# vaenyr/stable-diffusion-on-device

Hardware: AMD Instinct MI355X
Metric: images/sec + per-UNet-step ms, SD v1.4 512x512 20-step PLMS, 1/2/4/8 MI355X (higher is better)
Workload: dtype f16; 1 GPU; SD v1.4 txt2img 512x512, 20-step PLMS (21 UNet evals, batch 2 = cond+uncond per image), CLIP encode + VAE decode + uint8, guidance 7.5; images_per_gpu=1, global_batch=1, parallelism=dp1 (image shards, 1 RCCL broadcast), hip_graph=True, trajectory_graph=True, decode_overlaps_next_sampling=False

## Files before the change

include/sdod_engine.h:

```cpp
#ifndef SDOD_ENGINE_H
#define SDOD_ENGINE_H

#include <stddef.h>
#include <stdint.h>

#ifndef SDOD_API
#define SDOD_API
#endif

#ifdef __cplusplus
extern "C" {
#endif

enum sdod_graph_kind { SDOD_GRAPH_UNET = 0, SDOD_GRAPH_VAE_DECODER = 1, SDOD_GRAPH_TEXT_ENCODER = 2, SDOD_GRAPH_TEMB = 3,
                       SDOD_GRAPH_VAE_ENCODER = 4, SDOD_GRAPH_VAE_ENCODER_MASKED = 5 };

typedef struct sdod_model_config {
    int latent_channels;
    int latent_h;
    int latent_w;
    int model_channels;
    int context_dim;
    int context_len;
    int num_heads;
// ... 8 lines not shown
    int concat_channels;
} sdod_model_config;

SDOD_API void sdod_model_config_sd14(sdod_model_config* cfg);
SDOD_API void sdod_model_config_sd21(sdod_model_config* cfg);

SDOD_API int sdod_graph_create(void** graph, int kind, const sdod_model_config* cfg, int batch);
SDOD_API int sdod_graph_destroy(void* graph);

SDOD_API int sdod_graph_num_params(void* graph);
SDOD_API int sdod_graph_param_info(void* graph, int index, const char** name, int* ndim, int64_t shape[4]);
SDOD_API int sdod_graph_set_param(void* graph, const char* name, const void* data, int dtype, const int64_t* shape, int ndim);
SDOD_API int sdod_graph_param_device(void* graph, const char* name, void** device_ptr, size_t* bytes);
SDOD_API int sdod_graph_load_file(void* graph, const char* path, const char* prefix);
SDOD_API int sdod_graph_finalize(void* graph);
SDOD_API int sdod_graph_io(void* graph, int is_output, int index, void** device_ptr, size_t* bytes);
enum sdod_exec_flags { SDOD_EXEC_HIP_GRAPH = 1, SDOD_EXEC_STATIC_UNCHANGED = 2 };
SDOD_API int sdod_graph_execute(void* graph, void* stream, int flags);
SDOD_API int sdod_graph_check(void* graph);
SDOD_API int sdod_graph_num_ops(void* graph);
SDOD_API int sdod_graph_op_info(void* graph, int index, const char** label, double* flops, double* bytes);
SDOD_API int sdod_graph_op_detail(void* graph, int index, const char** detail);
SDOD_API int sdod_graph_profile(void* graph, void* stream, int iters, float* ms_out, int n);
SDOD_API int sdod_graph_stats(void* graph, size_t* weight_bytes, size_t* arena_bytes, int* num_launches, double* flops);
SDOD_API int sdod_graph_tune_info(void* graph, int* from_table, int* tuned_in_process, char* table_path, int cap);

#ifdef __cplusplus
}
#endif
#endif
// ... 1 lines not shown
```

include/sdod_hip.h:

```cpp
#ifndef SDOD_HIP_H
#define SDOD_HIP_H

#include <stddef.h>
#include <stdint.h>

#ifndef SDOD_API
#define SDOD_API
#endif

#ifdef __cplusplus
extern "C" {
#endif

enum sdod_act { SDOD_ACT_NONE = 0, SDOD_ACT_SILU = 1, SDOD_ACT_GELU = 2, SDOD_ACT_QUICK_GELU = 3 };
enum sdod_dtype { SDOD_F16 = 0, SDOD_F32 = 1, SDOD_U8Q = 2, SDOD_BF16 = 3  };
enum sdod_a_mode { SDOD_A_ROWS = 0, SDOD_A_CONV3X3 = 1  };

typedef struct sdod_gemm_desc {
    const void* a;
    const void* a2;
    const void* w;
    const void* bias;
    const void* row_bias;
    const void* residual;
// ... 181 lines not shown
    uint64_t seed, image_index0;
    int n, c, hw, uncond_first, mode, v_pred, last, noise_level, stage_reps, temb_width, temb_reps;
    float guidance, vc0, vc1, sqrt_one_minus_at, sqrt_at, sqrt_a_prev, dir_coef, known_sa, known_s1a;
} sdod_ddim_inpaint_step_args;
SDOD_API int sdod_ddim_inpaint_step(const sdod_ddim_inpaint_step_args* a, void* stream);
SDOD_API int sdod_mask_to_latent_f32(const uint8_t* mask_u8, float* keep, int n, int h_lat, int w_lat, int factor, void* stream);
SDOD_API int sdod_image_composite_u8(const void* img, const uint8_t* init_u8, const uint8_t* mask_u8, uint8_t* out_u8, int n, size_t hw,
                                     float a, float b, int mode, void* stream);
SDOD_API int sdod_image_to_u8(const void* img, uint8_t* out, size_t count, float a, float b, int mode, void* stream);

SDOD_API const char* sdod_hip_last_error(void);
SDOD_API int sdod_hip_device_info(int* cu_count, size_t* hbm_bytes, char* arch, int arch_len);

SDOD_API int sdod_l2_prefetch(const void* ptr, size_t bytes, void* stream);

#ifdef __cplusplus
}
#endif
#endif
```

stable-diffusion-on-device_amd/csrc/elementwise.hip:

```cpp
#include "common.h"
#include <atomic>
#include "sdod_hip.h"
#include "host_util.h"

#pragma clang fp contract(off)

namespace {

SDOD_DEVICE float mul_rn(float a, float b) { return a * b; }
SDOD_DEVICE float add_rn(float a, float b) { return a + b; }
SDOD_DEVICE float sub_rn(float a, float b) { return a - b; }
SDOD_DEVICE float div_rn(float a, float b) { return a / b; }

inline int grid_for(size_t work, int block = 256) {
    size_t b = (work + block - 1) / block;
    if (b > 2048) b = 2048;
    if (b < 1) b = 1;
    return (int)b;
}

#define GRID_STRIDE(i, n) \
    for (size_t i = (size_t)blockIdx.x * blockDim.x + threadIdx.x; i < (n); i += (size_t)gridDim.x * blockDim.x)

__global__ void geglu_kernel(const f16* x, f16* y, int M, int C) {
// ... 933 lines not shown
    SDOD_REQUIRE(out && e0 && count > 0 && div != 0.0f, "bad argument");
    LAUNCH(lincomb4_kernel, count, stream, out, e0, e1, e2, e3, c0, c1, c2, c3, div, count);
    return 0;
    SDOD_CATCH
}

extern "C" int sdod_image_to_u8(const void* img, uint8_t* out, size_t count, float a, float b, int mode, void* stream) {
    SDOD_TRY
    SDOD_REQUIRE(img && out && count > 0 && (mode == 0 || mode == 1), "bad argument");
    LAUNCH(to_u8_kernel, count, stream, (const f16*)img, out, count, a, b, mode);
    return 0;
    SDOD_CATCH
}

namespace {
__global__ __launch_bounds__(256) void l2_prefetch_kernel(const unsigned* __restrict__ p, size_t lines, unsigned* sink) {
    unsigned acc = 0;
    const size_t stride = (size_t)gridDim.x * blockDim.x;
    for (size_t i = (size_t)blockIdx.x * blockDim.x + threadIdx.x; i < lines; i += stride) acc += p[i * 32];
    if (acc == 0x9e3779b9u) *sink = acc;
}
}

extern "C" int sdod_l2_prefetch(const void* ptr, size_t bytes, void* stream) {
    SDOD_TRY
    SDOD_REQUIRE(ptr != nullptr && ((uintptr_t)ptr & 3) == 0, "null / unaligned pointer");
    const size_t lines = bytes / 128;
    if (lines == 0) return 0;
    static std::atomic<unsigned*> sink[64];
    int dev = 0;
// ... 16 lines not shown
```

stable-diffusion-on-device_amd/csrc/engine.h:

```cpp
#pragma once
#include <hip/hip_runtime.h>

#include <cstdint>
#include <functional>
#include <map>
#include <string>
#include <unordered_map>
#include <vector>

#include "host_util.h"
#include "sdod_engine.h"
#include "sdod_hip.h"

namespace sdod {

typedef _Float16 f16;

enum ParamKind {
    PK_CONV3,
    PK_CONV3_SMALL,
    PK_CONV1,
    PK_LINEAR,
    PK_EMBED,
    PK_VEC,
// ... 30 lines not shown
    void* ptr = nullptr;
    size_t bytes = 0;
};

class Graph {
public:
    Graph(int kind, const sdod_model_config& cfg, int batch);
    ~Graph();
    Graph(const Graph&) = delete;

    int num_params() const { return (int)params_.size(); }
    const Param& param(int i) const { return params_.at(i); }
    void set_param(const std::string& name, const void* data, int dtype, const int64_t* shape, int ndim);
    void load_file(const std::string& path, const std::string& prefix);
    void finalize();
    void execute(hipStream_t st, bool use_hip_graph, bool skip_static = false);
    void check_health() const;
    IoSlot io(bool output, int index) const;
    void stats(size_t* wbytes, size_t* abytes, int* launches, double* flops) const;

private:
    enum Mode { DECLARE, DRY, REAL };
    int kind_;
    sdod_model_config cfg_;
    int batch_;
    Mode mode_ = DECLARE;
    bool finalized_ = false;

    std::vector<Param> params_;
    std::unordered_map<std::string, int> pindex_;
    std::vector<std::vector<int>> groups_;
    std::unordered_map<std::string, int> gindex_;
    char* weight_base_ = nullptr;
    size_t weight_bytes_ = 0;
    float* qscale_ = nullptr;
    float* qoff_ = nullptr;
    size_t qrows_ = 0;
    bool quant_mode() const { return cfg_.weight_quant != 0 && (kind_ == SDOD_GRAPH_UNET || kind_ == SDOD_GRAPH_TEMB); }
    static constexpr int kQuantAutoMaxRows = 128;
    bool quant_decl_ = false;
    void quant_rows(int rows) { quant_decl_ = quant_mode() && (cfg_.weight_quant == 1 || rows <= kQuantAutoMaxRows); }
    void quant_global() { quant_decl_ = quant_mode(); }
// ... 89 lines not shown
        f16* c; const f16* p; int ld, n_out, n_mid, k;
        const float *bias_w, *bias_p;
        float* bias_out;
    };
    std::vector<ComposeJob> compose_jobs_;
    std::vector<void*> derived_;
    void emit_gemm(sdod_gemm_desc d);
    void linear(const f16* x, int rows, int K, int w, int N, f16* out, const GemmOpt& o);
    void linear_raw(const f16* x, int rows, int K, const f16* w, int ldw, int N, f16* out, const GemmOpt& o);
    Act conv(const Act& x, const Act* x2, int w, int cout, int ksize, int stride, bool upsample, const GemmOpt& o);
    Act group_norm(const Act& x, const Act* x2, int gw, int gb, float eps, bool silu);
    Act layer_norm(const Act& x, int lw, int lb, float eps);
    void attention(const f16* q, const f16* k, const f16* v, f16* out, int B, int heads, int lq, int lk, int d, int ldq,
                   int ldk, int ldv, int ldo, bool causal);

    Act res_block(const std::string& pfx, const Act& x, const Act* x2, int cout, const f16* emb_all, int emb_ld, int& emb_off);
    std::vector<Op>& sink() { return to_static_ ? static_ops_ : ops_; }
    struct PendingReduce {
        bool active = false;
        sdod_gemm_desc d{};
        double bytes = 0;
        std::string detail;
    } pending_;
    void flush_pending();
    std::vector<const void*> parked_;
    void release_after_consumer(const Act& a) { parked_.push_back(a.p); }
    void drain_parked() {
        for (const void* p : parked_) release(p);
        parked_.clear();
    }
    void settle() {
        flush_pending();
        drain_parked();
    }
    Act spatial_transformer(const std::string& pfx, const Act& x, const Act& ctx);
    Act vae_res_block(const std::string& pfx, const Act& x, int cout);
    Act vae_attn_block(const std::string& pfx, const Act& x);
    int emb_total_ = 0;
    int kv_total_ = 0;
    f16* kv_all_ = nullptr;
    int kv_off_ = 0;
    std::vector<std::pair<std::string, int>> unet_res_blocks() const;
    const char* group_base(const std::string& group) const;
    int group_first(const std::string& group) const;
    void emit(std::function<void(hipStream_t)> fn, const char* label = "elementwise", double flops = 0, double bytes = 0) {
        settle();
        if (mode_ == REAL) sink().push_back(Op{std::move(fn), label, flops, bytes, ""});
    }

public:
// ... 9 lines not shown
```

stable-diffusion-on-device_amd/csrc/engine.hip:

```cpp
#include "engine.h"

#include <cstdio>

#include <dlfcn.h>
#include <fcntl.h>
#include <sys/mman.h>
#include <sys/stat.h>
#include <unistd.h>

#include <algorithm>
#include <cstdlib>
#include <cstring>
#include <map>
#include <mutex>
#include <thread>

namespace sdod {

static inline size_t align_up(size_t v, size_t a) { return (v + a - 1) / a * a; }

static void check_rc(int rc) {
    if (rc != 0) throw Error(rc, get_last_error());
}

// ... 869 lines not shown
}

void Graph::build() {
    quant_global();
    switch (kind_) {
    case SDOD_GRAPH_UNET: build_unet(); break;
    case SDOD_GRAPH_VAE_DECODER: build_vae(); break;
    case SDOD_GRAPH_TEXT_ENCODER: build_clip(); break;
    case SDOD_GRAPH_VAE_ENCODER: build_vae_encoder(false); break;
    case SDOD_GRAPH_VAE_ENCODER_MASKED: build_vae_encoder(true); break;
    default: build_temb(); break;
    }
    settle();
}

void Graph::finalize() {
    allocate_weights();
    SDOD_REQUIRE(!finalized_, "graph already finalized");
    std::string missing;
    int nmiss = 0;
    for (auto& p : params_)
        if (!p.set) {
            if (nmiss < 5) missing += (nmiss ? ", " : "") + p.name;
            ++nmiss;
        }
    SDOD_REQUIRE(nmiss == 0, std::to_string(nmiss) + " parameter(s) not set: " + missing + (nmiss > 5 ? ", ..." : ""));
    mode_ = DRY;
    arena_reset();
    ws_need_ = gn_ws_need_ = 0;
    build();
// ... 244 lines not shown
    SDOD_TRY
    SDOD_REQUIRE(graph && path, "null argument");
    static_cast<Graph*>(graph)->load_file(path, prefix ? prefix : "");
    return 0;
    SDOD_CATCH
}

extern "C" int sdod_graph_finalize(void* graph) {
    SDOD_TRY
    SDOD_REQUIRE(graph != nullptr, "null graph");
    static_cast<Graph*>(graph)->finalize();
    return 0;
    SDOD_CATCH
}

extern "C" int sdod_graph_io(void* graph, int is_output, int index, void** device_ptr, size_t* bytes) {
    SDOD_TRY
    SDOD_REQUIRE(graph != nullptr, "null graph");
    const sdod::IoSlot s = static_cast<Graph*>(graph)->io(is_output != 0, index);
    if (device_ptr) *device_ptr = s.ptr;
    if (bytes) *bytes = s.bytes;
    return 0;
    SDOD_CATCH
}

extern "C" int sdod_graph_param_device(void* graph, const char* name, void** device_ptr, size_t* bytes) {
    SDOD_TRY
    SDOD_REQUIRE(graph != nullptr && name != nullptr, "null argument");
    Graph* g = static_cast<Graph*>(graph);
    for (int i = 0; i < g->num_params(); ++i) {
// ... 84 lines not shown
```

stable-diffusion-on-device_amd/csrc/graphs.hip:

```cpp
#include "engine.h"

namespace sdod {

static void check_rc2(int rc) {
    if (rc != 0) throw Error(rc, get_last_error());
}

int Graph::group_first(const std::string& group) const {
    auto it = gindex_.find(group);
    if (it == gindex_.end()) throw Error(INTERNAL_ERROR, "unknown parameter group " + group);
    return groups_[it->second].front();
}

const char* Graph::group_base(const std::string& group) const {
    auto it = gindex_.find(group);
    if (it == gindex_.end()) throw Error(INTERNAL_ERROR, "unknown parameter group " + group);
    return params_[groups_[it->second].front()].dev;
}

Act Graph::res_block(const std::string& pfx, const Act& x, const Act* x2, int cout, const f16* emb_all, int emb_ld, int& emb_off) {
    const int cin = x.c + (x2 ? x2->c : 0);
    quant_rows(x.rows());
    const int n1w = P(pfx + ".in_layers.0.weight", {cin}, PK_VEC), n1b = P(pfx + ".in_layers.0.bias", {cin}, PK_VEC);
    const int c1w = P(pfx + ".in_layers.2.weight", {cout, cin, 3, 3}, PK_CONV3), c1b = P(pfx + ".in_layers.2.bias", {cout}, PK_VEC);
    const int n2w = P(pfx + ".out_layers.0.weight", {cout}, PK_VEC), n2b = P(pfx + ".out_layers.0.bias", {cout}, PK_VEC);
    int c2w, skw = -1, skb = -1;
    const bool fuse_skip = !quant_decl_;
    if (cin != cout && !fuse_skip) {
        c2w = P(pfx + ".out_layers.3.weight", {cout, cout, 3, 3}, PK_CONV3);
        skw = P(pfx + ".skip_connection.weight", {cout, cin, 1, 1}, PK_CONV1);
        skb = P(pfx + ".skip_connection.bias", {cout}, PK_VEC);
    } else if (cin != cout) {
        const int ld = 9 * cout + cin;
        c2w = Pc(pfx + ".out_layers.3.weight", {cout, cout, 3, 3}, PK_CONV3, ld, 0, -1);
        skw = Pc(pfx + ".skip_connection.weight", {cout, cin, 1, 1}, PK_CONV1, ld, 9 * cout, c2w);
        skb = P(pfx + ".skip_connection.bias", {cout}, PK_VEC);
    } else {
// ... 4 lines not shown
    const int my_off = emb_off;
    emb_off += cout;

    Act g1 = group_norm(x, x2, n1w, n1b, 1e-5f, true);
    GemmOpt o1;
    o1.bias = c1b;
    o1.row_bias = emb_all ? emb_all + my_off : nullptr;
    o1.ld_row_bias = emb_ld;
    o1.rows_per_img = x.h * x.w;
    Act h = conv(g1, nullptr, c1w, cout, 3, 1, false, o1);
    release(g1);
    Act g2 = group_norm(h, nullptr, n2w, n2b, 1e-5f, true);
    release(h);
    GemmOpt o2;
    o2.bias = c2b;
    Act sk;
    if (cin != cout && !fuse_skip) {
        GemmOpt os;
        os.bias = skb;
        sk = conv(x, x2, skw, cout, 1, 1, false, os);
        o2.residual = sk.p;
    } else if (cin != cout) {
        o2.tail0 = &x;
        o2.tail1 = x2;
        o2.bias2 = skb;
    } else {
        if (x2) throw Error(INTERNAL_ERROR, "identity skip with a concatenated input");
        o2.residual = x.p;
    }
    Act out = conv(g2, nullptr, c2w, cout, 3, 1, false, o2);
    release(g2);
    if (sk.p) release_after_consumer(sk);
    return out;
}

Act Graph::spatial_transformer(const std::string& pfx, const Act& x, const Act& ctx) {
    const int C = x.c, cd = ctx.c;
    const int heads = cfg_.num_heads > 0 ? cfg_.num_heads : C / cfg_.head_dim;
    const int d = C / heads;
    const int rows = x.rows(), L = x.h * x.w, B = x.n;
    const std::string tb = pfx + ".transformer_blocks.0";
    quant_rows(rows);
    const bool quant_block = quant_decl_;
    const int nw = P(pfx + ".norm.weight", {C}, PK_VEC), nb = P(pfx + ".norm.bias", {C}, PK_VEC);
    const bool lin = cfg_.linear_proj != 0;
    const int piw = lin ? P(pfx + ".proj_in.weight", {C, C}, PK_LINEAR) : P(pfx + ".proj_in.weight", {C, C, 1, 1}, PK_CONV1);
    const int pib = P(pfx + ".proj_in.bias", {C}, PK_VEC);
    const int l1w = P(tb + ".norm1.weight", {C}, PK_VEC), l1b = P(tb + ".norm1.bias", {C}, PK_VEC);
    const std::string gq = tb + ".attn1.qkv";
    P(tb + ".attn1.to_q.weight", {C, C}, PK_LINEAR, gq);
    P(tb + ".attn1.to_k.weight", {C, C}, PK_LINEAR, gq);
// ... 13 lines not shown
    static const bool compose_on = [] { const char* e = std::getenv("SDOD_COMPOSE"); return !(e && e[0] == '0'); }();
    const bool compose = compose_on && !quant_block;
    int f2w, pow_;
    if (compose) {
        f2w = Pc(tb + ".ff.net.2.weight", {C, 4 * C}, PK_LINEAR, 5 * C, 0, -1);
        pow_ = lin ? Pc(pfx + ".proj_out.weight", {C, C}, PK_LINEAR, 5 * C, 4 * C, f2w)
                   : Pc(pfx + ".proj_out.weight", {C, C, 1, 1}, PK_CONV1, 5 * C, 4 * C, f2w);
    } else {
        f2w = P(tb + ".ff.net.2.weight", {C, 4 * C}, PK_LINEAR);
        pow_ = lin ? P(pfx + ".proj_out.weight", {C, C}, PK_LINEAR) : P(pfx + ".proj_out.weight", {C, C, 1, 1}, PK_CONV1);
    }
    const int f2b = P(tb + ".ff.net.2.bias", {C}, PK_VEC);
    const int pob = P(pfx + ".proj_out.bias", {C}, PK_VEC);
    if (mode_ == DECLARE) return act(x.n, x.h, x.w, C);

    Act g = group_norm(x, nullptr, nw, nb, 1e-6f, false);
    Act t0 = act(B, 1, L, C);
    { GemmOpt o; o.bias = pib; linear(g.p, rows, C, piw, C, t0.p, o); }
    release(g);
    const bool fold = !quant_block;
    auto normed = [&](const Act& src, int lw, int lb) -> Act { return layer_norm(src, lw, lb, 1e-5f); };
    f16* qkv = alloc((size_t)rows * 3 * C);
    if (fold) {
        GemmOpt o; o.ln_w = l1w; o.ln_b = l1b;
        linear_raw(t0.p, rows, C, reinterpret_cast<const f16*>(group_base(gq)), C, 3 * C, qkv, o);
    } else {
        Act nrm = normed(t0, l1w, l1b);
        GemmOpt o; o.wq_scale = qscale_of(group_first(gq)); o.wq_off = qoff_of(group_first(gq));
        linear_raw(nrm.p, rows, C, reinterpret_cast<const f16*>(group_base(gq)), C, 3 * C, qkv, o);
        release(nrm);
    }
    f16* a1 = alloc((size_t)rows * C);
    attention(qkv, qkv + C, qkv + 2 * C, a1, B, heads, L, L, d, 3 * C, 3 * C, 3 * C, C, false);
    release(qkv);
    Act t1 = act(B, 1, L, C);
    { GemmOpt o; o.bias = o1b; o.residual = t0.p; linear(a1, rows, C, o1w, C, t1.p, o); }
    release(a1); release(t0);
    static const bool xfold_on = [] { const char* e = std::getenv("SDOD_XATTN_FOLD"); return !(e && e[0] == '0'); }();
    const int NK = heads * 80;
    const bool xfold = xfold_on && fold && ctx.w <= 80 && NK % 320 == 0 && L % 32 == 0 && d <= 160 && d % 4 == 0;
    if (xfold) {
        f16 *w1 = nullptr, *w2 = nullptr;
        float *s1 = nullptr, *t1v = nullptr;
        f16* wq = reinterpret_cast<f16*>(params_[q2w].dev);
        const f16* wo = reinterpret_cast<const f16*>(params_[o2w].dev);
        if (mode_ == REAL) {
            SDOD_HIP_CHECK(hipMalloc((void**)&w1, (size_t)B * NK * C * sizeof(f16)));
            SDOD_HIP_CHECK(hipMalloc((void**)&w2, (size_t)B * NK * C * sizeof(f16)));
            SDOD_HIP_CHECK(hipMalloc((void**)&s1, (size_t)B * NK * sizeof(float)));
            SDOD_HIP_CHECK(hipMalloc((void**)&t1v, (size_t)B * NK * sizeof(float)));
            derived_.push_back(w1); derived_.push_back(w2); derived_.push_back(s1); derived_.push_back(t1v);
            const LnVecs qv = ln_fold_vectors(wq, C, C, C, l2w, l2b, nullptr);
// ... 161 lines not shown
                              "M" + std::to_string(B * H * Wd) + " N" + std::to_string(MC) + " K64"});
        }
    } else {
        f16* cols = alloc((size_t)B * H * Wd * 64);
        emit([=](hipStream_t st) { check_rc2(sdod_latent_im2col_f16(x_in, cols, B, H, Wd, LC, 64, 1.0f, st)); });
        { GemmOpt o; o.bias = cib; linear(cols, B * H * Wd, 64, ciw, MC, h.p, o); }
        release(cols);
    }

    std::vector<Act> hs;
    hs.push_back(h);
    int ch = MC, ds = 1, idx = 1;
    for (int level = 0; level < 4; ++level) {
        for (int i = 0; i < 2; ++i) {
            const std::string pfx = "input_blocks." + std::to_string(idx++);
            Act r = res_block(pfx + ".0", h, nullptr, mult[level] * MC, emb_all, emb_ld, emb_off);
            ch = mult[level] * MC;
            if (ds <= 4) {
                Act t = spatial_transformer(pfx + ".1", r, ctx);
                release(r);
                r = t;
            }
            h = r;
            hs.push_back(h);
        }
        if (level != 3) {
            const std::string pfx = "input_blocks." + std::to_string(idx++) + ".0.op";
            quant_rows(h.rows() / 4);
            const int w = P(pfx + ".weight", {ch, ch, 3, 3}, PK_CONV3), b = P(pfx + ".bias", {ch}, PK_VEC);
            GemmOpt o; o.bias = b;
            h = conv(h, nullptr, w, ch, 3, 2, false, o);
            hs.push_back(h);
            ds *= 2;
        }
// ... 356 lines not shown
```

stable-diffusion-on-device_amd/csrc/libsdod/context.cpp:

```cpp
#include "context.h"

#include <algorithm>
#include <cstdio>
#include <cstring>

#include "sdod_hip.h"

namespace sdod {

static void rc_check(int rc) {
    if (rc != 0) throw Error(rc, get_last_error());
}

void Logger::log(LogLevel l, const std::string& msg) const {
    if (l == LogLevel::NOTHING || (unsigned)l > (unsigned)level_) return;
    static const char* tag[] = {"", "E", "I", "D", "A"};
    std::FILE* sink = l == LogLevel::ERROR ? stderr : stdout;
    std::fprintf(sink, "[libsdod %s] %s\n", tag[(unsigned)l], msg.c_str());
    std::fflush(sink);
}

namespace {
struct Timer {
    std::chrono::steady_clock::time_point t0 = std::chrono::steady_clock::now();
// ... 30 lines not shown
    Timer t;
    tokenizer_.emplace(models_dir_ + "/ctokenizer.txt");
    logger_.info("Tokenizer created!");
    solver_.emplace(1000, 0.00085f, 0.0120f);
    logger_.info("ODE solver prepared!");
    SDOD_HIP_CHECK(hipSetDevice(device_));
    SDOD_HIP_CHECK(hipStreamCreateWithFlags(&stream_, hipStreamNonBlocking));

    struct Item { std::unique_ptr<Graph>* slot; int kind; int batch; const char* stem; };
    const Item items[] = {{&unet_, SDOD_GRAPH_UNET, 2, "unet"}, {&text_, SDOD_GRAPH_TEXT_ENCODER, 1, "text_encoder"},
                          {&vae_, SDOD_GRAPH_VAE_DECODER, 1, "vae_decoder"}};
    for (const Item& it : items) {
        logger_.info(std::string("Attempting to load a model: ") + it.stem + ".sdodw");
        it.slot->reset(new Graph(it.kind, cfg_, it.batch));
        (*it.slot)->load_file(weight_path(it.stem), "");
        (*it.slot)->finalize();
        logger_.info(std::string("Model ") + it.stem + " loaded");
    }
    logger_.info("All models loaded!");

    const size_t lat = (size_t)latent_channels_ * latent_spatial_ * latent_spatial_;
    SDOD_HIP_CHECK(hipMalloc((void**)&x_dev_, 2 * lat * sizeof(float)));
    SDOD_HIP_CHECK(hipMalloc((void**)&e_dev_, lat * sizeof(float)));
    SDOD_HIP_CHECK(hipMalloc((void**)&y_prev_, lat * sizeof(float)));
    SDOD_HIP_CHECK(hipMalloc((void**)&img_u8_, image_bytes()));
    SDOD_HIP_CHECK(hipMalloc((void**)&ctx_uncond_, (size_t)cfg_.context_len * cfg_.context_dim * sizeof(f16)));
    x_host_.resize(lat);

    encode_prompt("", ctx_uncond_);
    logger_.info("Input/output buffers created and prepared!");
// ... 129 lines not shown
```

stable-diffusion-on-device_amd/csrc/norms.hip:

```cpp
#include "common.h"
#include "sdod_hip.h"
#include "host_util.h"

#include <algorithm>
#include <cstdlib>

namespace {

struct GnMom {
    float n, mean, m2;
};
SDOD_DEVICE GnMom gn_merge(GnMom a, const GnMom& b) {
    if (b.n == 0.f) return a;
    if (a.n == 0.f) return b;
    const float n = a.n + b.n, d = b.mean - a.mean, f = b.n / n;
    a.mean += d * f;
    a.m2 += b.m2 + d * d * a.n * f;
    a.n = n;
    return a;
}

template <typename T>
struct Chunk8;
template <>
// ... 951 lines not shown
            if (pix < pix_end) {
                f16x8 o;
#pragma unroll
                for (int e = 0; e < 8; ++e) {
                    float f = (float)v[k][e] * s8[e] + t8[e];
                    if (p.silu) f = silu_f(f);
                    o[e] = (f16)f;
                }
                stg8(p.y + (row0 + pix) * p.C + c0, o);
            }
        }
    }
}

constexpr size_t GN_GRID_MIN_BYTES = (size_t)5 << 20;

static int gn_device_cus() {
    static std::atomic<int> cus[64];
    int dev = 0;
    if (hipGetDevice(&dev) != hipSuccess || dev < 0 || dev >= 64) return 0;
    int v = cus[dev].load(std::memory_order_relaxed);
    if (v == 0) {
        if (hipDeviceGetAttribute(&v, hipDeviceAttributeMultiprocessorCount, dev) != hipSuccess || v <= 0) v = -1;
        cus[dev].store(v, std::memory_order_relaxed);
    }
    return v > 0 ? v : 0;
}

static int gn_grid_plan(int n, int hw, int c0, int c1, int groups, GnGridP* out) {
    const int c = c0 + c1;
    if (groups > 32 || n <= 0 || !gn2_fits(c0, c1, groups) || c / 8 > 512) return 0;
    if ((size_t)n * hw * c * 2 < GN_GRID_MIN_BYTES) return 0;
    int cus = gn_device_cus();
    if (cus > 256) cus = 256;
    const int wpi = cus / n;
    if (wpi < 8 || wpi > GN_MAX_CHUNKS_GRID) return 0;
    const int cp = c / 8, rp = 512 / cp;
    const int ppw = (hw + wpi - 1) / wpi;
    const int k = (ppw + rp - 1) / rp;
    if (k > 16 * 8) return 0;
    if (out) {
        out->cp = cp; out->rp = rp; out->wpi = wpi; out->ppw = ppw; out->nwg = wpi * n;
        out->nloop = k <= 16 ? 1 : (k + 15) / 16;
    }
    return k <= 4 ? 4 : k <= 8 ? 8 : 16;
}

// ... 726 lines not shown
```

stable-diffusion-on-device_amd/sdod/amd/_lib.py:

```python
import ctypes
import os

_HERE = os.path.dirname(os.path.abspath(__file__))
LIB_DIR = os.path.normpath(os.path.join(_HERE, '..', '..', 'lib'))

_cache = {}


def load(name):
    if name in _cache:
        return _cache[name]
    path = os.path.join(LIB_DIR, os.environ.get('SDOD_LIBSDOD', name) if name == 'libsdod.so' else name)
    if not os.path.exists(path):
        raise ImportError(
            f'{path} not found: build the MI355X extension first '
            f'(python -c "import __graft_entry__ as g; g.build()" or make -C stable-diffusion-on-device_amd). '
            f'There is no CPU fallback for the HIP path.')
    lib = ctypes.CDLL(path, mode=ctypes.RTLD_GLOBAL)
    _cache[name] = lib
    return lib


class SdodError(RuntimeError):
    def __init__(self, code, msg):
# ... 105 lines not shown
        'sdod_ddim_inpaint_step': (c_int, [ctypes.POINTER(DdimInpaintStepArgs), P]),
        'sdod_mask_to_latent_f32': (c_int, [P, P, c_int, c_int, c_int, c_int, P]),
        'sdod_image_composite_u8': (c_int, [P, P, P, P, c_int, c_size_t, c_float, c_float, c_int, P]),
        'sdod_nchw_f32_to_nhwc_f16': (c_int, [P, P, c_int, c_int, c_int, c_float, P]),
        'sdod_nhwc_f16_to_nchw_f32': (c_int, [P, P, c_int, c_int, c_int, P]),
        'sdod_latent_prep_f16': (c_int, [P, P, P, P, c_int, c_int, c_int, c_float, P]),
        'sdod_embedding_f16': (c_int, [P, P, P, P, c_int, c_int, c_int, P]),
        'sdod_timestep_features_f16': (c_int, [P, P, c_int, c_int, P]),
        'sdod_stage_unet_inputs': (c_int, [P, P, c_size_t, c_int, P, P, c_size_t, c_int, P]),
        'sdod_randn_f32': (c_int, [P, P, c_size_t, ctypes.c_uint64, ctypes.c_uint64, P]),
        'sdod_cfg_combine': (c_int, [P, P, c_int, c_int, c_int, c_float, c_int, c_int, P]),
        'sdod_dpm_update': (c_int, [P, P, P, c_size_t, c_int, c_float, c_float, c_float, c_float, c_float, P]),
        'sdod_ddim_step_f32': (c_int, [P, P, c_size_t, c_float, c_float, c_float, c_float, P]),
        'sdod_lincomb4_f32': (c_int, [P, P, P, P, P, c_float, c_float, c_float, c_float, c_float, c_size_t, P]),
        'sdod_image_to_u8': (c_int, [P, P, c_size_t, c_float, c_float, c_int, P]),
        'sdod_hip_last_error': (c_char_p, []),
        'sdod_hip_device_info': (c_int, [ctypes.POINTER(c_int), ctypes.POINTER(c_size_t), c_char_p, c_int]),
    }
    for name, (res, args) in sig.items():
        fn = getattr(lib, name)
        fn.restype = res
        fn.argtypes = args


HIP_SYMBOLS = [
    'sdod_gemm_f16', 'sdod_gemm_fixup', 'sdod_gemm_fixup_counters', 'sdod_gemm_workspace_bytes', 'sdod_gemm_plan', 'sdod_gemm_halo_ok', 'sdod_gemm_panel_ok', 'sdod_gemm_xcd_panels', 'sdod_gemm_num_tiles', 'sdod_gemm_tile_shape', 'sdod_gemm_tile_info', 'sdod_gemm_time', 'sdod_gemm_time_cold', 'sdod_group_norm_workspace_bytes', 'sdod_group_norm_layout', 'sdod_group_norm_status', 'sdod_group_norm_clear_error', 'sdod_l2_prefetch', 'sdod_group_norm_launches', 'sdod_group_norm_path', 'sdod_group_norm_nhwc', 'sdod_group_norm_nchw', 'sdod_group_norm_nchw_workspace_bytes', 'sdod_gemm_reduce_info', 'sdod_group_norm_reduce_ok', 'sdod_group_norm_reduce_nhwc',
    'sdod_layer_norm_f16', 'sdod_ln_fold_f16', 'sdod_compose_linear_f16', 'sdod_attention_f16', 'sdod_xattn_fold_f16', 'sdod_softmax_rows_f16', 'sdod_geglu_f16', 'sdod_act_f16',
    'sdod_add_f16', 'sdod_concat_channels_f16', 'sdod_im2col3x3_small_f16', 'sdod_latent_im2col_f16', 'sdod_conv_in_f16', 'sdod_image_conv_in_f16', 'sdod_conv_in_cat_f16', 'sdod_masked_image_conv_in_f16', 'sdod_inpaint_cond_f32', 'sdod_encode_latent_f32', 'sdod_plms_update', 'sdod_dpm_step', 'sdod_ddim_inpaint_step', 'sdod_mask_to_latent_f32', 'sdod_image_composite_u8', 'sdod_nchw_f32_to_nhwc_f16',
    'sdod_nhwc_f16_to_nchw_f32', 'sdod_latent_prep_f16', 'sdod_embedding_f16', 'sdod_timestep_features_f16', 'sdod_cfg_combine', 'sdod_stage_unet_inputs', 'sdod_randn_f32',
    'sdod_dpm_update', 'sdod_ddim_step_f32', 'sdod_lincomb4_f32', 'sdod_image_to_u8', 'sdod_hip_last_error',
    'sdod_hip_device_info',
]


def check(code):
    if code != 0:
        msg = hip().sdod_hip_last_error()
        raise SdodError(code, msg.decode() if msg else 'unknown error')
```

stable-diffusion-on-device_amd/sdod/amd/engine.py:

```python
import contextlib
import ctypes

import numpy as np
import torch

from . import _lib
from ._lib import check

UNET, VAE_DECODER, TEXT_ENCODER, TEMB, VAE_ENCODER, VAE_ENCODER_MASKED = 0, 1, 2, 3, 4, 5


class ModelConfig(ctypes.Structure):
    _fields_ = [(n, ctypes.c_int) for n in (
        'latent_channels', 'latent_h', 'latent_w', 'model_channels', 'context_dim', 'context_len', 'num_heads',
        'head_dim', 'vocab_size', 'text_layers', 'text_heads', 'vae_channels', 'linear_proj', 'text_arch', 'weight_quant',
        'concat_channels')]


ENGINE_SYMBOLS = [
    'sdod_model_config_sd14', 'sdod_model_config_sd21', 'sdod_graph_create', 'sdod_graph_destroy', 'sdod_graph_num_params', 'sdod_graph_param_info',
    'sdod_graph_set_param', 'sdod_graph_param_device', 'sdod_graph_load_file', 'sdod_graph_finalize', 'sdod_graph_io', 'sdod_graph_execute', 'sdod_graph_check',
    'sdod_graph_stats', 'sdod_graph_tune_info', 'sdod_graph_num_ops', 'sdod_graph_op_info', 'sdod_graph_op_detail', 'sdod_graph_profile',
]


def _engine():
    lib = _lib.hip()
    if not getattr(lib, '_sdod_engine_typed', False):
        P, I = ctypes.c_void_p, ctypes.c_int
        lib.sdod_model_config_sd14.argtypes = [ctypes.POINTER(ModelConfig)]
        lib.sdod_model_config_sd14.restype = None
        lib.sdod_model_config_sd21.argtypes = [ctypes.POINTER(ModelConfig)]
        lib.sdod_model_config_sd21.restype = None
        lib.sdod_graph_create.argtypes = [ctypes.POINTER(P), I, ctypes.POINTER(ModelConfig), I]
        lib.sdod_graph_destroy.argtypes = [P]
        lib.sdod_graph_num_params.argtypes = [P]
        lib.sdod_graph_param_info.argtypes = [P, I, ctypes.POINTER(ctypes.c_char_p), ctypes.POINTER(I), ctypes.POINTER(ctypes.c_int64)]
        lib.sdod_graph_set_param.argtypes = [P, ctypes.c_char_p, P, I, ctypes.POINTER(ctypes.c_int64), I]
        lib.sdod_graph_load_file.argtypes = [P, ctypes.c_char_p, ctypes.c_char_p]
        lib.sdod_graph_param_device.argtypes = [P, ctypes.c_char_p, ctypes.POINTER(P), ctypes.POINTER(ctypes.c_size_t)]
        lib.sdod_graph_finalize.argtypes = [P]
        lib.sdod_graph_io.argtypes = [P, I, I, ctypes.POINTER(P), ctypes.POINTER(ctypes.c_size_t)]
        lib.sdod_graph_execute.argtypes = [P, P, I]
        lib.sdod_graph_check.argtypes = [P]
        lib.sdod_graph_stats.argtypes = [P, ctypes.POINTER(ctypes.c_size_t), ctypes.POINTER(ctypes.c_size_t), ctypes.POINTER(I),
                                         ctypes.POINTER(ctypes.c_double)]
        lib.sdod_graph_tune_info.argtypes = [P, ctypes.POINTER(I), ctypes.POINTER(I), ctypes.c_char_p, I]
        lib.sdod_graph_num_ops.argtypes = [P]
        lib.sdod_graph_op_info.argtypes = [P, I, ctypes.POINTER(ctypes.c_char_p), ctypes.POINTER(ctypes.c_double), ctypes.POINTER(ctypes.c_double)]
        lib.sdod_graph_profile.argtypes = [P, P, I, P, I]
        lib.sdod_graph_op_detail.argtypes = [P, I, ctypes.POINTER(ctypes.c_char_p)]
        lib._sdod_engine_typed = True
    return lib


def sd14_config(latent_h=64, latent_w=64, concat_channels=0):
# ... 69 lines not shown
        check(self._lib.sdod_graph_param_device(self._h, name.encode(), ctypes.byref(p), ctypes.byref(n)))
        return device_view(p.value, (n.value // torch.empty((), dtype=dtype).element_size(),), dtype, self.device)

    def load_state_dict(self, sd, prefix=''):
        with torch.cuda.device(self.device):
            for name, _ in self.param_table():
                key = prefix + name
                if key not in sd:
                    raise KeyError(f'missing parameter {key}')
                self.set_param(name, sd[key])

    def load_file(self, path, prefix=''):
        with self._on_device():
            check(self._lib.sdod_graph_load_file(self._h, path.encode(), prefix.encode()))

    def finalize(self):
        with torch.cuda.device(self.device):
            check(self._lib.sdod_graph_finalize(self._h))
        self.finalized = True
        return self

    def _io(self, is_out, idx):
        p = ctypes.c_void_p(); n = ctypes.c_size_t()
        check(self._lib.sdod_graph_io(self._h, 1 if is_out else 0, idx, ctypes.byref(p), ctypes.byref(n)))
        return p.value, n.value

    def io_tensor(self, is_out, idx, shape, dtype):
        ptr, nbytes = self._io(is_out, idx)
        numel = int(np.prod(shape))
        assert numel * torch.empty((), dtype=dtype).element_size() == nbytes, (shape, dtype, nbytes)
# ... 123 lines not shown
```

stable-diffusion-on-device_amd/sdod/amd/pipeline.py:

```python
import numpy as np
import torch

from . import engine as E
from . import ops
from .host import DpmSolver
from .samplers import PLMS_ORDERS, PlmsSchedule


class Txt2Img:
    inpaint_unet = False
    _cond_staged = False
    encoder = None
    masked_encoder = None
    _traj = None

    def __init__(self, state_dicts=None, models_dir=None, images_per_gpu=1, latent_hw=64, device='cuda:0', use_hip_graph=True,
                 tokenizer=None, with_text_encoder=True, model='sd14', with_vae=True, cfg_split=False, weight_quant=None,
                 with_vae_encoder=False, inpaint_unet=False):
        self.device = torch.device(device)
        torch.cuda.set_device(self.device)
        self.n = images_per_gpu
        self.model = model
        self.v_prediction = model == 'sd21'
        self.cfg = E.sd21_config(latent_hw, latent_hw) if model == 'sd21' else E.sd14_config(latent_hw, latent_hw)
# ... 8 lines not shown
        self._pair = None
        if self.cfg_split:
            import torch.distributed as dist
            if not (dist.is_available() and dist.is_initialized() and dist.get_world_size() % 2 == 0):
                raise RuntimeError('cfg_split needs torch.distributed initialised with an even world size')
            rank = dist.get_rank()
            self._half = rank % 2
            for a in range(0, dist.get_world_size(), 2):
                grp = dist.new_group([a, a + 1])
                if a == rank - self._half:
                    self._pair = grp
            self._pair_staged = dist.get_backend() == 'gloo'
        self.use_hip_graph = use_hip_graph
        self.tokenizer = tokenizer
        self.unet = E.UNet(self.cfg, self.n if cfg_split else 2 * self.n, device)
        self.vae = E.VaeDecoder(self.cfg, 1, device) if with_vae else None
        self.text = E.TextEncoder(self.cfg, 2, device) if with_text_encoder else None
        self.encoder = E.VaeEncoder(self.cfg, 1, device) if with_vae_encoder else None
        self.masked_encoder = E.MaskedVaeEncoder(self.cfg, 1, device) if self.inpaint_unet else None
        self._temb_graphs = {}
        self._sd = state_dicts
        self._dir = models_dir
        for g, key, stem in ((self.unet, 'unet', 'unet'), (self.vae, 'vae', 'vae_decoder'), (self.text, 'text', 'text_encoder'),
                             (self.encoder, 'vae_enc', 'vae_encoder'), (self.masked_encoder, 'vae_enc', 'vae_encoder')):
            if g is None:
                continue
            self._load(g, key, stem)
            g.finalize()
        self._temb_cache = {}
        self._ctx_fresh = True
# ... 451 lines not shown
```

Baseline: 10.82 images/s.

## Share cond/uncond computation in first UNet res block and self-attention prefix

Adds a paired-batch mode to the UNet graph. In the first input block, the res block and the transformer's group norm, proj_in, self-attention and out projection run only on half the batch, because the cond and uncond rows see the same latent and timestep. The results are then copied to the other half with a new pair_broadcast kernel. This removes duplicated work at the highest-resolution level, at the cost of an extra copy kernel. It relies on both CFG halves having identical inputs up to the cross-attention. The mode is on by default and can be turned off with an environment variable; a group-norm grid threshold also becomes an environment override.

```diff
diff --git a/include/sdod_engine.h b/include/sdod_engine.h
--- a/include/sdod_engine.h
+++ b/include/sdod_engine.h
@@ -46,6 +46,7 @@
 SDOD_API int sdod_graph_param_device(void* graph, const char* name, void** device_ptr, size_t* bytes);
 SDOD_API int sdod_graph_load_file(void* graph, const char* path, const char* prefix);
 SDOD_API int sdod_graph_finalize(void* graph);
+SDOD_API int sdod_graph_set_paired_batch(void* graph, int on);
 SDOD_API int sdod_graph_io(void* graph, int is_output, int index, void** device_ptr, size_t* bytes);
 enum sdod_exec_flags { SDOD_EXEC_HIP_GRAPH = 1, SDOD_EXEC_STATIC_UNCHANGED = 2 };
 SDOD_API int sdod_graph_execute(void* graph, void* stream, int flags);
diff --git a/include/sdod_hip.h b/include/sdod_hip.h
--- a/include/sdod_hip.h
+++ b/include/sdod_hip.h
@@ -219,6 +219,8 @@
 
 SDOD_API int sdod_l2_prefetch(const void* ptr, size_t bytes, void* stream);
 
+SDOD_API int sdod_pair_broadcast(const void* src0, void* dst0, size_t bytes0, const void* src1, void* dst1, size_t bytes1, void* stream);
+
 #ifdef __cplusplus
 }
 #endif
diff --git a/stable-diffusion-on-device_amd/csrc/elementwise.hip b/stable-diffusion-on-device_amd/csrc/elementwise.hip
--- a/stable-diffusion-on-device_amd/csrc/elementwise.hip
+++ b/stable-diffusion-on-device_amd/csrc/elementwise.hip
@@ -971,6 +971,28 @@
 }
 
 namespace {
+__global__ __launch_bounds__(256) void pair_broadcast_kernel(const u32x4* __restrict__ s0, u32x4* __restrict__ d0, size_t n0,
+                                                             const u32x4* __restrict__ s1, u32x4* __restrict__ d1, size_t n1) {
+    GRID_STRIDE(i, n0 + n1) {
+        if (i < n0) d0[i] = s0[i];
+        else d1[i - n0] = s1[i - n0];
+    }
+}
+}
+
+extern "C" int sdod_pair_broadcast(const void* src0, void* dst0, size_t bytes0, const void* src1, void* dst1, size_t bytes1, void* stream) {
+    SDOD_TRY
+    SDOD_REQUIRE(src0 && dst0 && bytes0 > 0 && bytes0 % 16 == 0 && (((uintptr_t)src0 | (uintptr_t)dst0) & 15) == 0,
+                 "first pair: non-null 16-byte aligned pointers and a positive multiple of 16 bytes");
+    SDOD_REQUIRE(bytes1 == 0 || (src1 && dst1 && bytes1 % 16 == 0 && (((uintptr_t)src1 | (uintptr_t)dst1) & 15) == 0),
+                 "second pair: 16-byte aligned pointers and a multiple of 16 bytes (or 0 bytes)");
+    LAUNCH(pair_broadcast_kernel, (bytes0 + bytes1) / 16, stream, (const u32x4*)src0, (u32x4*)dst0, bytes0 / 16, (const u32x4*)src1, (u32x4*)dst1,
+           bytes1 / 16);
+    return 0;
+    SDOD_CATCH
+}
+
+namespace {
 __global__ __launch_bounds__(256) void l2_prefetch_kernel(const unsigned* __restrict__ p, size_t lines, unsigned* sink) {
     unsigned acc = 0;
     const size_t stride = (size_t)gridDim.x * blockDim.x;
diff --git a/stable-diffusion-on-device_amd/csrc/engine.h b/stable-diffusion-on-device_amd/csrc/engine.h
--- a/stable-diffusion-on-device_amd/csrc/engine.h
+++ b/stable-diffusion-on-device_amd/csrc/engine.h
@@ -68,6 +68,7 @@
     void set_param(const std::string& name, const void* data, int dtype, const int64_t* shape, int ndim);
     void load_file(const std::string& path, const std::string& prefix);
     void finalize();
+    void set_paired_batch(bool on);
     void execute(hipStream_t st, bool use_hip_graph, bool skip_static = false);
     void check_health() const;
     IoSlot io(bool output, int index) const;
@@ -80,6 +81,7 @@
     int batch_;
     Mode mode_ = DECLARE;
     bool finalized_ = false;
+    bool paired_ = false;
 
     std::vector<Param> params_;
     std::unordered_map<std::string, int> pindex_;
@@ -199,7 +201,8 @@
     void attention(const f16* q, const f16* k, const f16* v, f16* out, int B, int heads, int lq, int lk, int d, int ldq,
                    int ldk, int ldv, int ldo, bool causal);
 
-    Act res_block(const std::string& pfx, const Act& x, const Act* x2, int cout, const f16* emb_all, int emb_ld, int& emb_off);
+    Act res_block(const std::string& pfx, const Act& x, const Act* x2, int cout, const f16* emb_all, int emb_ld, int& emb_off,
+                  f16* out = nullptr);
     std::vector<Op>& sink() { return to_static_ ? static_ops_ : ops_; }
     struct PendingReduce {
         bool active = false;
@@ -218,7 +221,7 @@
         flush_pending();
         drain_parked();
     }
-    Act spatial_transformer(const std::string& pfx, const Act& x, const Act& ctx);
+    Act spatial_transformer(const std::string& pfx, const Act& x, const Act& ctx, bool pair_prefix = false);
     Act vae_res_block(const std::string& pfx, const Act& x, int cout);
     Act vae_attn_block(const std::string& pfx, const Act& x);
     int emb_total_ = 0;
diff --git a/stable-diffusion-on-device_amd/csrc/engine.hip b/stable-diffusion-on-device_amd/csrc/engine.hip
--- a/stable-diffusion-on-device_amd/csrc/engine.hip
+++ b/stable-diffusion-on-device_amd/csrc/engine.hip
@@ -907,6 +907,14 @@
     settle();
 }
 
+void Graph::set_paired_batch(bool on) {
+    SDOD_REQUIRE(kind_ == SDOD_GRAPH_UNET, "paired batch is a mode of the UNET graph");
+    SDOD_REQUIRE(batch_ % 2 == 0, "paired batch needs an even batch (rows b and b + B/2 form a pair), got " + std::to_string(batch_));
+    SDOD_REQUIRE(!finalized_, "paired batch must be chosen before finalize() (the launch list is built there)");
+    static const bool share_on = [] { const char* e = std::getenv("SDOD_CFG_SHARE"); return !(e && e[0] == '0'); }();
+    paired_ = on && share_on;
+}
+
 void Graph::finalize() {
     allocate_weights();
     SDOD_REQUIRE(!finalized_, "graph already finalized");
@@ -1181,6 +1189,14 @@
     SDOD_CATCH
 }
 
+extern "C" int sdod_graph_set_paired_batch(void* graph, int on) {
+    SDOD_TRY
+    SDOD_REQUIRE(graph != nullptr, "null graph");
+    static_cast<Graph*>(graph)->set_paired_batch(on != 0);
+    return 0;
+    SDOD_CATCH
+}
+
 extern "C" int sdod_graph_io(void* graph, int is_output, int index, void** device_ptr, size_t* bytes) {
     SDOD_TRY
     SDOD_REQUIRE(graph != nullptr, "null graph");
diff --git a/stable-diffusion-on-device_amd/csrc/graphs.hip b/stable-diffusion-on-device_amd/csrc/graphs.hip
--- a/stable-diffusion-on-device_amd/csrc/graphs.hip
+++ b/stable-diffusion-on-device_amd/csrc/graphs.hip
@@ -18,9 +18,9 @@
     return params_[groups_[it->second].front()].dev;
 }
 
-Act Graph::res_block(const std::string& pfx, const Act& x, const Act* x2, int cout, const f16* emb_all, int emb_ld, int& emb_off) {
+Act Graph::res_block(const std::string& pfx, const Act& x, const Act* x2, int cout, const f16* emb_all, int emb_ld, int& emb_off, f16* out_to) {
     const int cin = x.c + (x2 ? x2->c : 0);
-    quant_rows(x.rows());
+    quant_rows(out_to ? x.h * x.w * batch_ : x.rows());
     const int n1w = P(pfx + ".in_layers.0.weight", {cin}, PK_VEC), n1b = P(pfx + ".in_layers.0.bias", {cin}, PK_VEC);
     const int c1w = P(pfx + ".in_layers.2.weight", {cout, cin, 3, 3}, PK_CONV3), c1b = P(pfx + ".in_layers.2.bias", {cout}, PK_VEC);
     const int n2w = P(pfx + ".out_layers.0.weight", {cout}, PK_VEC), n2b = P(pfx + ".out_layers.0.bias", {cout}, PK_VEC);
@@ -55,6 +55,7 @@
     release(h);
     GemmOpt o2;
     o2.bias = c2b;
+    o2.out = out_to;
     Act sk;
     if (cin != cout && !fuse_skip) {
         GemmOpt os;
@@ -75,7 +76,7 @@
     return out;
 }
 
-Act Graph::spatial_transformer(const std::string& pfx, const Act& x, const Act& ctx) {
+Act Graph::spatial_transformer(const std::string& pfx, const Act& x, const Act& ctx, bool pair_prefix) {
     const int C = x.c, cd = ctx.c;
     const int heads = cfg_.num_heads > 0 ? cfg_.num_heads : C / cfg_.head_dim;
     const int d = C / heads;
@@ -119,28 +120,40 @@
     const int pob = P(pfx + ".proj_out.bias", {C}, PK_VEC);
     if (mode_ == DECLARE) return act(x.n, x.h, x.w, C);
 
-    Act g = group_norm(x, nullptr, nw, nb, 1e-6f, false);
-    Act t0 = act(B, 1, L, C);
-    { GemmOpt o; o.bias = pib; linear(g.p, rows, C, piw, C, t0.p, o); }
+    const int PB = pair_prefix ? B / 2 : B, prows = PB * L;
+    Act xh = x;
+    xh.n = PB;
+    Act g = group_norm(xh, nullptr, nw, nb, 1e-6f, false);
+    Act t0 = act(PB, 1, L, C);
+    { GemmOpt o; o.bias = pib; linear(g.p, prows, C, piw, C, t0.p, o); }
     release(g);
     const bool fold = !quant_block;
     auto normed = [&](const Act& src, int lw, int lb) -> Act { return layer_norm(src, lw, lb, 1e-5f); };
-    f16* qkv = alloc((size_t)rows * 3 * C);
+    f16* qkv = alloc((size_t)prows * 3 * C);
     if (fold) {
         GemmOpt o; o.ln_w = l1w; o.ln_b = l1b;
-        linear_raw(t0.p, rows, C, reinterpret_cast<const f16*>(group_base(gq)), C, 3 * C, qkv, o);
+        linear_raw(t0.p, prows, C, reinterpret_cast<const f16*>(group_base(gq)), C, 3 * C, qkv, o);
     } else {
         Act nrm = normed(t0, l1w, l1b);
         GemmOpt o; o.wq_scale = qscale_of(group_first(gq)); o.wq_off = qoff_of(group_first(gq));
-        linear_raw(nrm.p, rows, C, reinterpret_cast<const f16*>(group_base(gq)), C, 3 * C, qkv, o);
+        linear_raw(nrm.p, prows, C, reinterpret_cast<const f16*>(group_base(gq)), C, 3 * C, qkv, o);
         release(nrm);
     }
-    f16* a1 = alloc((size_t)rows * C);
-    attention(qkv, qkv + C, qkv + 2 * C, a1, B, heads, L, L, d, 3 * C, 3 * C, 3 * C, C, false);
+    f16* a1 = alloc((size_t)prows * C);
+    attention(qkv, qkv + C, qkv + 2 * C, a1, PB, heads, L, L, d, 3 * C, 3 * C, 3 * C, C, false);
     release(qkv);
     Act t1 = act(B, 1, L, C);
-    { GemmOpt o; o.bias = o1b; o.residual = t0.p; linear(a1, rows, C, o1w, C, t1.p, o); }
+    { GemmOpt o; o.bias = o1b; o.residual = t0.p; linear(a1, prows, C, o1w, C, t1.p, o); }
     release(a1); release(t0);
+    if (pair_prefix) {
+        const size_t half = (size_t)prows * C;
+        const f16* xs = x.p; f16* xd = x.p + half;
+        const f16* ts = t1.p; f16* td = t1.p + half;
+        settle();
+        if (mode_ == REAL)
+            ops_.push_back(Op{[=](hipStream_t st) { check_rc2(sdod_pair_broadcast(xs, xd, half * sizeof(f16), ts, td, half * sizeof(f16), st)); },
+                              "pair_broadcast", 0, 4.0 * half * sizeof(f16), "2 x m" + std::to_string(prows) + " c" + std::to_string(C)});
+    }
     static const bool xfold_on = [] { const char* e = std::getenv("SDOD_XATTN_FOLD"); return !(e && e[0] == '0'); }();
     const int NK = heads * 80;
     const bool xfold = xfold_on && fold && ctx.w <= 80 && NK % 320 == 0 && L % 32 == 0 && d <= 160 && d % 4 == 0;
@@ -332,10 +345,19 @@
     for (int level = 0; level < 4; ++level) {
         for (int i = 0; i < 2; ++i) {
             const std::string pfx = "input_blocks." + std::to_string(idx++);
-            Act r = res_block(pfx + ".0", h, nullptr, mult[level] * MC, emb_all, emb_ld, emb_off);
+            const bool pair = paired_ && mode_ != DECLARE && level == 0 && i == 0;
+            Act r;
+            if (pair) {
+                r = act(B, h.h, h.w, mult[level] * MC);
+                Act hh = h;
+                hh.n = B / 2;
+                res_block(pfx + ".0", hh, nullptr, mult[level] * MC, emb_all, emb_ld, emb_off, r.p);
+            } else {
+                r = res_block(pfx + ".0", h, nullptr, mult[level] * MC, emb_all, emb_ld, emb_off);
+            }
             ch = mult[level] * MC;
             if (ds <= 4) {
-                Act t = spatial_transformer(pfx + ".1", r, ctx);
+                Act t = spatial_transformer(pfx + ".1", r, ctx, pair);
                 release(r);
                 r = t;
             }
diff --git a/stable-diffusion-on-device_amd/csrc/libsdod/context.cpp b/stable-diffusion-on-device_amd/csrc/libsdod/context.cpp
--- a/stable-diffusion-on-device_amd/csrc/libsdod/context.cpp
+++ b/stable-diffusion-on-device_amd/csrc/libsdod/context.cpp
@@ -68,6 +68,7 @@
         logger_.info(std::string("Attempting to load a model: ") + it.stem + ".sdodw");
         it.slot->reset(new Graph(it.kind, cfg_, it.batch));
         (*it.slot)->load_file(weight_path(it.stem), "");
+        if (it.kind == SDOD_GRAPH_UNET) (*it.slot)->set_paired_batch(true);
         (*it.slot)->finalize();
         logger_.info(std::string("Model ") + it.stem + " loaded");
     }
diff --git a/stable-diffusion-on-device_amd/csrc/norms.hip b/stable-diffusion-on-device_amd/csrc/norms.hip
--- a/stable-diffusion-on-device_amd/csrc/norms.hip
+++ b/stable-diffusion-on-device_amd/csrc/norms.hip
@@ -989,6 +989,13 @@
 }
 
 constexpr size_t GN_GRID_MIN_BYTES = (size_t)5 << 20;
+static size_t gn_grid_min_bytes() {
+    static const size_t v = [] {
+        const char* e = std::getenv("SDOD_GN_GRID_MIN");
+        return e && e[0] ? (size_t)std::strtoull(e, nullptr, 10) : GN_GRID_MIN_BYTES;
+    }();
+    return v;
+}
 
 static int gn_device_cus() {
     static std::atomic<int> cus[64];
@@ -1005,7 +1012,7 @@
 static int gn_grid_plan(int n, int hw, int c0, int c1, int groups, GnGridP* out) {
     const int c = c0 + c1;
     if (groups > 32 || n <= 0 || !gn2_fits(c0, c1, groups) || c / 8 > 512) return 0;
-    if ((size_t)n * hw * c * 2 < GN_GRID_MIN_BYTES) return 0;
+    if ((size_t)n * hw * c * 2 < gn_grid_min_bytes()) return 0;
     int cus = gn_device_cus();
     if (cus > 256) cus = 256;
     const int wpi = cus / n;
diff --git a/stable-diffusion-on-device_amd/sdod/amd/_lib.py b/stable-diffusion-on-device_amd/sdod/amd/_lib.py
--- a/stable-diffusion-on-device_amd/sdod/amd/_lib.py
+++ b/stable-diffusion-on-device_amd/sdod/amd/_lib.py
@@ -143,6 +143,7 @@
         'sdod_ddim_step_f32': (c_int, [P, P, c_size_t, c_float, c_float, c_float, c_float, P]),
         'sdod_lincomb4_f32': (c_int, [P, P, P, P, P, c_float, c_float, c_float, c_float, c_float, c_size_t, P]),
         'sdod_image_to_u8': (c_int, [P, P, c_size_t, c_float, c_float, c_int, P]),
+        'sdod_pair_broadcast': (c_int, [P, P, c_size_t, P, P, c_size_t, P]),
         'sdod_hip_last_error': (c_char_p, []),
         'sdod_hip_device_info': (c_int, [ctypes.POINTER(c_int), ctypes.POINTER(c_size_t), c_char_p, c_int]),
     }
@@ -158,7 +159,7 @@
     'sdod_add_f16', 'sdod_concat_channels_f16', 'sdod_im2col3x3_small_f16', 'sdod_latent_im2col_f16', 'sdod_conv_in_f16', 'sdod_image_conv_in_f16', 'sdod_conv_in_cat_f16', 'sdod_masked_image_conv_in_f16', 'sdod_inpaint_cond_f32', 'sdod_encode_latent_f32', 'sdod_plms_update', 'sdod_dpm_step', 'sdod_ddim_inpaint_step', 'sdod_mask_to_latent_f32', 'sdod_image_composite_u8', 'sdod_nchw_f32_to_nhwc_f16',
     'sdod_nhwc_f16_to_nchw_f32', 'sdod_latent_prep_f16', 'sdod_embedding_f16', 'sdod_timestep_features_f16', 'sdod_cfg_combine', 'sdod_stage_unet_inputs', 'sdod_randn_f32',
     'sdod_dpm_update', 'sdod_ddim_step_f32', 'sdod_lincomb4_f32', 'sdod_image_to_u8', 'sdod_hip_last_error',
-    'sdod_hip_device_info',
+    'sdod_hip_device_info', 'sdod_pair_broadcast',
 ]
 
 
diff --git a/stable-diffusion-on-device_amd/sdod/amd/engine.py b/stable-diffusion-on-device_amd/sdod/amd/engine.py
--- a/stable-diffusion-on-device_amd/sdod/amd/engine.py
+++ b/stable-diffusion-on-device_amd/sdod/amd/engine.py
@@ -21,6 +21,7 @@
     'sdod_model_config_sd14', 'sdod_model_config_sd21', 'sdod_graph_create', 'sdod_graph_destroy', 'sdod_graph_num_params', 'sdod_graph_param_info',
     'sdod_graph_set_param', 'sdod_graph_param_device', 'sdod_graph_load_file', 'sdod_graph_finalize', 'sdod_graph_io', 'sdod_graph_execute', 'sdod_graph_check',
     'sdod_graph_stats', 'sdod_graph_tune_info', 'sdod_graph_num_ops', 'sdod_graph_op_info', 'sdod_graph_op_detail', 'sdod_graph_profile',
+    'sdod_graph_set_paired_batch',
 ]
 
 
@@ -40,6 +41,7 @@
         lib.sdod_graph_load_file.argtypes = [P, ctypes.c_char_p, ctypes.c_char_p]
         lib.sdod_graph_param_device.argtypes = [P, ctypes.c_char_p, ctypes.POINTER(P), ctypes.POINTER(ctypes.c_size_t)]
         lib.sdod_graph_finalize.argtypes = [P]
+        lib.sdod_graph_set_paired_batch.argtypes = [P, I]
         lib.sdod_graph_io.argtypes = [P, I, I, ctypes.POINTER(P), ctypes.POINTER(ctypes.c_size_t)]
         lib.sdod_graph_execute.argtypes = [P, P, I]
         lib.sdod_graph_check.argtypes = [P]
@@ -139,6 +141,10 @@
         with self._on_device():
             check(self._lib.sdod_graph_load_file(self._h, path.encode(), prefix.encode()))
 
+    def set_paired_batch(self, on=True):
+        check(self._lib.sdod_graph_set_paired_batch(self._h, 1 if on else 0))
+        return self
+
     def finalize(self):
         with torch.cuda.device(self.device):
             check(self._lib.sdod_graph_finalize(self._h))
diff --git a/stable-diffusion-on-device_amd/sdod/amd/pipeline.py b/stable-diffusion-on-device_amd/sdod/amd/pipeline.py
--- a/stable-diffusion-on-device_amd/sdod/amd/pipeline.py
+++ b/stable-diffusion-on-device_amd/sdod/amd/pipeline.py
@@ -46,6 +46,8 @@
         self.use_hip_graph = use_hip_graph
         self.tokenizer = tokenizer
         self.unet = E.UNet(self.cfg, self.n if cfg_split else 2 * self.n, device)
+        if not cfg_split:
+            self.unet.set_paired_batch(True)
         self.vae = E.VaeDecoder(self.cfg, 1, device) if with_vae else None
         self.text = E.TextEncoder(self.cfg, 2, device) if with_text_encoder else None
         self.encoder = E.VaeEncoder(self.cfg, 1, device) if with_vae_encoder else None
```

Result: no change. 10.83 images/s, median of 3 (+0.1%).
